# zhaoyuhsin/Edge-Guided-Near-Eye-Image-Analysis-for-Head-Mounted-Displays

Hardware: AMD Instinct MI355X
Metric: eye-frames/sec (320x240): inference edge+seg (value), +fit, exact fp32, and train fwd+bwd at 1 MI355X (higher is better)
Workload: dtype f32 tensors; inference products split into f16 hi/lo pairs (3 f16 MFMAs per product, 22-bit significand), f32 accumulate (`exact_fp32`: every product on the f32 MFMA); `train`: bf16 storage, f32 accumulate, f32 master weights (and an f32-storage leg)

## Files before the change

### edge-guided-near-eye-image-analysis-for-head-mounted-displays_amd/_lib.py

```python
import ctypes as C
import os

_HERE = os.path.dirname(os.path.abspath(__file__))
LIB_PATH = os.environ.get("EGNE_LIB") or os.path.join(_HERE, "csrc", "libegne_hip.so")

MAXSEG, MAXGROUP = 8, 3
ACT_NONE, ACT_RELU, ACT_LEAKY = 0, 1, 2

c_fp = C.c_void_p


class Seg(C.Structure):
    _fields_ = [("ptr", c_fp), ("pix_stride", C.c_int64), ("ch_off", C.c_int32), ("Cp", C.c_int32),
                ("scale", c_fp), ("shift", c_fp), ("act_in", C.c_int32), ("presplit", C.c_int32)]


class ConvDesc(C.Structure):
    _fields_ = [("B", C.c_int32), ("H", C.c_int32), ("W", C.c_int32), ("Ho", C.c_int32), ("Wo", C.c_int32),
                ("kh", C.c_int32), ("kw", C.c_int32), ("stride", C.c_int32),
                ("pad_h", C.c_int32), ("pad_w", C.c_int32), ("pad_mode", C.c_int32),
                ("ngroups", C.c_int32), ("dil", C.c_int32 * MAXGROUP),
                ("nseg", C.c_int32), ("seg", Seg * MAXSEG),
                ("Ktot", C.c_int32), ("CoutP", C.c_int32),
                ("w", c_fp), ("bias", c_fp), ("act", C.c_int32),
                ("post_scale", c_fp), ("post_shift", c_fp),
                ("residual", c_fp), ("res_pix_stride", C.c_int64), ("res_ch_off", C.c_int32),
                ("out", c_fp), ("out_pix_stride", C.c_int64), ("out_ch_off", C.c_int32),
                ("Cout_store", C.c_int32),
                ("stats_ws", c_fp), ("stats_nchunk", C.c_int32),
                ("pool_out", c_fp), ("pool_pix_stride", C.c_int64), ("pool_ch_off", C.c_int32),
                ("dyn_scale", C.c_void_p), ("absmax_out", C.c_void_p), ("dtype", C.c_int32),
                ("out_split", C.c_int32), ("out_split_scale", C.c_float), ("ovf_flag", C.c_void_p), ("f16_products", C.c_int32),
                ("mask_y", C.c_void_p), ("mask_pix_stride", C.c_int64), ("mask_ch_off", C.c_int32), ("mask_act", C.c_int32), ("mask_sums", C.c_void_p)]


class Dst(C.Structure):
    _fields_ = [("out", C.c_void_p), ("out_pix_stride", C.c_int64), ("out_ch_off", C.c_int32), ("C", C.c_int32), ("CoutP", C.c_int32),
                ("wfrag", C.c_void_p), ("residual", C.c_void_p), ("res_pix_stride", C.c_int64), ("res_ch_off", C.c_int32),
                ("mask_y", C.c_void_p), ("mask_pix_stride", C.c_int64), ("mask_ch_off", C.c_int32), ("act", C.c_int32),
                ("sums", C.c_void_p), ("res_pixels", C.c_int64)]


MAXDST = 6


class ConvQuery(C.Structure):
    _fields_ = [("dtype", C.c_int32), ("B", C.c_int32), ("H", C.c_int32), ("W", C.c_int32),
                ("kh", C.c_int32), ("kw", C.c_int32), ("stride", C.c_int32), ("pad_h", C.c_int32), ("pad_w", C.c_int32), ("pad_mode", C.c_int32),
                ("ngroups", C.c_int32), ("dil", C.c_int32 * MAXGROUP), ("nseg", C.c_int32),
                ("seg_C", C.c_int32 * MAXSEG), ("seg_Cp", C.c_int32 * MAXSEG), ("seg_ch_off", C.c_int32 * MAXSEG), ("seg_pix_stride", C.c_int64 * MAXSEG),
                ("seg_affine", C.c_int32 * MAXSEG), ("seg_planar", C.c_int32), ("seg_presplit", C.c_int32),
                ("Cout", C.c_int32), ("Cout_store", C.c_int32), ("dst_Cp", C.c_int32), ("dst_ch_off", C.c_int32), ("dst_pix_stride", C.c_int64),
                ("act", C.c_int32), ("has_post", C.c_int32), ("has_residual", C.c_int32), ("res_pix_stride", C.c_int64), ("res_ch_off", C.c_int32),
                ("split", C.c_int32), ("split1", C.c_int32), ("split_c4", C.c_int32), ("train", C.c_int32), ("dyn_scales", C.c_int32),
                ("is_dgrad", C.c_int32), ("want_stats", C.c_int32), ("want_pool", C.c_int32), ("pool_Cp", C.c_int32), ("pool_pix_stride", C.c_int64),
                ("want_scores", C.c_int32), ("up_add", C.c_int32), ("narrow_bf16_ok", C.c_int32), ("f16_products", C.c_int32), ("f16_storage", C.c_int32)]


class ConvChoice(C.Structure):
    _fields_ = [("kind", C.c_int32), ("name", C.c_char * 32), ("tail_frames", C.c_int32), ("fused_stats", C.c_int32), ("fused_pool", C.c_int32),
                ("small_ws_floats", C.c_int64)]


class BdcnTailDesc(C.Structure):
    _fields_ = [("B", C.c_int32), ("H", C.c_int32), ("W", C.c_int32),
                ("s", c_fp * 5), ("s1", c_fp * 5), ("h", C.c_int32 * 5), ("w", C.c_int32 * 5),
                ("stride", C.c_int32 * 5), ("crop", C.c_int32 * 5), ("up", c_fp * 5),
                ("fuse_w", c_fp), ("fuse_b", c_fp), ("out", c_fp * 11), ("edge_thres", C.c_int32)]


class LossDesc(C.Structure):
    _fields_ = [("B", C.c_int32), ("H", C.c_int32), ("W", C.c_int32),
                ("logits", c_fp), ("pix_stride", C.c_int64), ("ch_off", C.c_int32),
                ("target", c_fp), ("spatWts", c_fp), ("distMap", c_fp), ("cond", c_fp),
                ("pupil_center", c_fp), ("elNorm", c_fp), ("elOut", c_fp), ("alpha", C.c_float),
                ("grid_x", c_fp), ("grid_y", c_fp),
                ("partials", c_fp), ("out_terms", c_fp), ("pred_c", c_fp), ("elPred", c_fp),
                ("mask", c_fp), ("op_nchw", c_fp), ("coef", c_fp), ("dtype", C.c_int32),
                ("g_op_nchw", c_fp), ("g_pred_c", c_fp), ("g_elOut_up", c_fp)]


i32, i64, f32, vp = C.c_int32, C.c_int64, C.c_float, C.c_void_p
SIGNATURES = {
    "egne_conv2d_fwd": (i32, [C.POINTER(ConvDesc), vp]),
    "egne_pack_conv_weight": (i32, [vp, i32, i32, i32, i32, vp, i32, i32, vp, vp]),
    "egne_pack_conv_weight_frag": (i32, [vp, i32, i32, i32, i32, vp, i32, i32, vp, vp]),
    "egne_conv3x3_halo_supported": (i32, [C.POINTER(ConvDesc)]),
    "egne_conv3x3_halo_fwd": (i32, [C.POINTER(ConvDesc), vp]),
    "egne_conv3x3_smallcin_fwd": (i32, [C.POINTER(ConvDesc), vp, vp]),
    "egne_pack_conv_weight_f16x2": (i32, [vp, i32, i32, i32, i32, i32, i32, f32, vp, vp, vp]),
    "egne_conv2d_f16x3_fwd": (i32, [C.POINTER(ConvDesc), vp, vp, f32, f32, vp]),
    "egne_conv2d_f16x3_small_workspace_floats": (i64, [C.POINTER(ConvDesc)]),
    "egne_conv2d_f16x3_small_fwd": (i32, [C.POINTER(ConvDesc), vp, vp, f32, f32, vp, i64, vp]),
    "egne_pack_conv_weight_f16frag": (i32, [vp, i32, i32, i32, i32, i32, i32, f32, vp, vp, vp]),
    "egne_conv3x3_halo_f16_fwd": (i32, [C.POINTER(ConvDesc), vp, vp, f32, f32, vp]),
    "egne_conv1x1_3x3_fused_f16_fwd": (i32, [C.POINTER(ConvDesc), C.POINTER(ConvDesc), vp, vp, f32, f32, vp, vp, f32, f32, vp]),
    "egne_conv3x3c4_3x3_fused_f16_fwd": (i32, [C.POINTER(ConvDesc), C.POINTER(ConvDesc), vp, vp, f32, f32, vp, vp, f32, f32, vp]),
    "egne_msblock_dil_scores_f16_fwd": (i32, [C.POINTER(ConvDesc), vp, vp, f32, f32, vp, vp, vp, vp, i32, vp]),
    "egne_msblock_dil_f16_fwd": (i32, [C.POINTER(ConvDesc), vp, vp, f32, f32, vp]),
    "egne_conv3x3_rs_f16_fwd": (i32, [C.POINTER(ConvDesc), vp, vp, f32, f32, vp]),
    "egne_conv3x3_rw_f16_fwd": (i32, [C.POINTER(ConvDesc), vp, vp, f32, f32, vp]),
    "egne_conv1x1_pool2_f16x3_fwd": (i32, [C.POINTER(ConvDesc), vp, vp, f32, f32, vp]),
    "egne_conv1x1_f16x3_fwd": (i32, [C.POINTER(ConvDesc), vp, vp, f32, f32, vp]),
    "egne_dist_maps_workspace_bytes": (i64, [i32, i32, i32, i32]),
    "egne_dist_maps": (i32, [vp, i32, i32, i32, i32, vp, vp, vp]),
    "egne_zscore": (i32, [vp, vp, i32, i32, vp]),
    "egne_spatial_weights": (i32, [vp, i32, i32, i32, vp, vp]),
    "egne_eval_prep_workspace_bytes": (i64, [i32, i32, i32, i32, i32]),
    "egne_eval_prep": (i32, [vp, i32, i32, i32, i32, i32, i32, i32, vp, vp, vp, vp, i32, i32, vp, vp, vp, vp]),
    "egne_eval_render": (i32, [vp, i32, i32, i32, i32, i32, vp, vp, vp, i32, i32, C.c_double, i32, vp, vp, vp, vp, vp]),
    "egne_jpeg_workspace_bytes": (i64, [i32, i32, i32]),
    "egne_jpeg_encode": (i32, [vp, i32, i32, i32, vp, vp, vp, vp, i32, i32, vp, i64, vp, vp, vp, vp]),
    "egne_stamp_mask": (i32, [vp, i32, i32, i32, vp, i32, i32, i32, i32, i32, i32, i32, vp]),
    "egne_jpeg_decode_workspace_bytes": (i64, [i32, i32, i32, i32, i64, i32, i32]),
    "egne_jpeg_decode": (i32, [vp, i64, vp, i32, i32, i32, i32, i32, i32, vp, vp, vp, vp, vp, vp]),
    "egne_deepvog_loss_workspace_floats": (i64, [i32, i32, i32]),
    "egne_deepvog_loss_fwd": (i32, [vp, i64, i32, vp, vp, vp, i32, i32, i32, vp, vp, vp, vp, vp, vp]),
    "egne_deepvog_loss_bwd": (i32, [vp, i64, i32, vp, vp, vp, i32, i32, i32, vp, vp, vp, vp, i64, i32, vp]),
    "egne_affine_act": (i32, [vp, i64, i32, vp, i64, i32, i32, i64, vp, vp, i32, vp]),
    "egne_augment": (i32, [vp, vp, vp, vp, vp, vp, vp, vp, i32, i32, i32, vp]),
    "egne_augment_cv": (i32, [vp, vp, vp, vp, vp, vp, vp, vp, vp, vp, i32, i32, i32, vp]),
    "egne_loader_stage": (i32, [vp, vp, vp, i32, i32, i32, i32, i32, i32, i32, vp, vp, vp, vp, vp, vp, vp, vp, vp]),
    "egne_loader_finish": (i32, [vp, vp, vp, vp, i32, i32, vp]),
    "egne_conv3x3_smallcin_f16_fwd": (i32, [C.POINTER(ConvDesc), vp, vp, f32, f32, vp]),
    "egne_pack_conv3x3_c4_weight_f16": (i32, [vp, i32, i32, i32, f32, vp, vp, vp]),
    "egne_conv1x1_ms_f16x3_fwd": (i32, [C.POINTER(ConvDesc), vp, vp, f32, f32, vp]),
    "egne_pack_conv1x1_weight_f16x2_map": (i32, [vp, i32, i32, vp, i32, i32, f32, vp, vp, vp]),
    "egne_conv2d_f16x3_big_fwd": (i32, [C.POINTER(ConvDesc), vp, f32, f32, vp]),
    "egne_pack_conv_weight_f16img": (i32, [vp, i32, i32, i32, i32, i32, i32, f32, vp, vp]),
    "egne_conv2d_f16_big1_fwd": (i32, [C.POINTER(ConvDesc), vp, f32, f32, vp]),
    "egne_conv2d_f16_big1_supported": (i32, [C.POINTER(ConvDesc)]),
    "egne_pack_conv_weight_f16img1": (i32, [vp, i32, i32, i32, i32, i32, i32, f32, vp, vp]),
    "egne_pack_conv1x1_weight_f16": (i32, [vp, i32, i32, vp, i32, i32, f32, vp, vp, vp]),
    "egne_absmax": (i32, [vp, i64, i32, i32, i64, vp, vp]),
    "egne_absmax_f16": (i32, [vp, i64, i32, i32, i64, vp, vp]),
    "egne_norm_stats_workspace_bytes": (i64, [i32, i32, i32, i32]),
    "egne_norm_stats": (i32, [vp, i64, i32, i32, i32, i32, i32, f32, vp, vp, vp, vp, vp, vp]),
    "egne_norm_stats_finish": (i32, [vp, i32, i32, i32, i32, f32, vp, vp, vp]),
    "egne_norm_stats_finish_moments": (i32, [vp, i32, i32, i32, i32, f32, vp, vp, vp, vp, vp]),
    "egne_affine_inplace": (i32, [vp, i64, i32, i32, i64, vp, vp, vp]),
    "egne_affine": (i32, [vp, i64, i32, vp, i64, i32, i32, i64, vp, vp, vp]),
    "egne_avgpool2": (i32, [vp, i64, i32, vp, i64, i32, i32, i32, i32, i32, vp]),
    "egne_norm_act_pool2": (i32, [vp, i64, i32, vp, vp, i32, vp, i64, i32, i32, i32, i32, i32, vp]),
    "egne_maxpool2": (i32, [vp, i64, i32, vp, i64, i32, i32, i32, i32, i32, i32, i32, i32, vp]),
    "egne_maxpool2_f16": (i32, [vp, i64, i32, vp, i64, i32, i32, i32, i32, i32, i32, i32, i32, vp]),
    "egne_maxpool2_split": (i32, [vp, i64, i32, vp, i64, i32, i32, i32, i32, i32, i32, i32, i32, vp]),
    "egne_upsample2x": (i32, [vp, i64, i32, vp, i64, i32, i32, i32, i32, i32, vp]),
    "egne_upsample2x_nearest": (i32, [vp, i64, i32, vp, i64, i32, i32, i32, i32, i32, vp]),
    "egne_upsample2x_nearest_bwd": (i32, [vp, i64, i32, vp, i64, i32, i32, i32, i32, i32, vp]),
    "egne_nchw_to_nhwc": (i32, [vp, i32, i32, i32, i32, vp, i64, i32, i32, vp]),
    "egne_nhwc_to_nchw": (i32, [vp, i64, i32, i32, i32, i32, i32, vp, vp]),
    "egne_bdcn_stage_scores": (i32, [C.POINTER(vp), i32, i64, i64, vp, vp, vp, vp, vp, vp, vp, vp, vp]),
    "egne_bdcn_tail": (i32, [C.POINTER(BdcnTailDesc), vp]),
    "egne_loss_workspace_floats": (i64, [i32, i32, i32]),
    "egne_loss_fwd": (i32, [C.POINTER(LossDesc), vp]),
    "egne_selfcorr_workspace_floats": (i64, [i32, i32, i32]),
    "egne_selfcorr_fwd": (i32, [C.POINTER(LossDesc), f32, vp, vp, vp]),
    "egne_selfcorr_bwd": (i32, [C.POINTER(LossDesc), f32, vp, vp, vp, vp, vp, vp]),
    "egne_ellipse_head_act": (i32, [vp, i32, i32, vp]),
    "egne_selu_inplace": (i32, [vp, i64, vp]),
    "egne_spatial_mean": (i32, [vp, i64, i32, i32, i32, i32, vp, vp]),
    "egne_softmax3": (i32, [vp, i64, i32, vp, i64, i32, i32, i64, vp]),
    "egne_adain": (i32, [vp, i64, i32, i32, vp, vp, i64, i32, vp, i64, i32, i32, i32, f32, vp]),
    "egne_conf_loss": (i32, [vp, i32, vp, i32, i32, i32, f32, vp, vp]),
    "egne_loss_bwd": (i32, [C.POINTER(LossDesc), vp, vp, i64, i32, vp, vp]),
    "egne_act_bwd_bias_workspace_bytes": (i64, [i64, i32]),
    "egne_act_bwd_bias": (i32, [vp, i64, i32, vp, i64, i32, i32, i32, i64, vp, i32, i32, vp, vp]),
    "egne_act_bwd_bias_absmax": (i32, [vp, i64, i32, vp, i64, i32, i32, i32, i64, vp, i32, i32, vp, vp, vp]),
    "egne_act_norm_bwd": (i32, [vp, i64, i32, vp, i64, i32, i32, vp, vp, vp, i64, i32, vp, i64, i32, i32, i32, i32, i32, i32, vp, vp, vp, i32, vp, i32, vp]),
    "egne_bn_act_bwd": (i32, [vp, i64, i32, i32, vp, vp, vp, vp, i64, i32, i32, i32, i32, i32, vp, i64, i32, vp, vp, vp, vp, i32, vp, i32, vp, vp]),
    "egne_zero_many": (i32, [vp, i32, i64, vp]),
    "egne_pair_bias_bwd_workspace_bytes": (i64, [i32, i32]),
    "egne_pair_bias_bwd": (i32, [vp, i64, i32, i32, i32, i32, i32, vp, vp, i32, i32, vp, vp, vp, vp]),
    "egne_norm_bwd_workspace_bytes": (i64, [i32, i32, i32, i32]),
# ... 92 lines not shown
```

### edge-guided-near-eye-image-analysis-for-head-mounted-displays_amd/csrc/conv_f16x3.hip

```cpp
#include "common.h"
#include "kernel_util.h"
#include "split_f16.h"
#include <cstdlib>

namespace {

constexpr int KC = 32;
constexpr int LDH = 40;

__device__ __forceinline__ float act_apply(float v, int act) {
  if (act == EGNE_ACT_RELU) return fmaxf(v, 0.f);
  if (act == EGNE_ACT_LEAKY) return v > 0.f ? v : 0.01f * v;
  return v;
}

template <int WGM, int WGN, int TM, int TN, bool GROUPED, int PS = 0>
__global__ __launch_bounds__(256) void conv_f16x3_kernel(const egne_conv_desc p, const _Float16* __restrict__ whi,
                                                         const _Float16* __restrict__ wlo, float a_scale,
                                                         float out_scale, float* __restrict__ ksplit_ws) {
  egne::dyn_scales(p.dyn_scale, a_scale, out_scale);
  constexpr int BM = WGM * TM * 32, BN = WGN * TN * 32;
  constexpr int AR = BM / 32;
  constexpr int BI = (BN * 4 + 255) / 256;
  __shared__ __attribute__((aligned(16))) _Float16 lds[(2 * BM + 2 * BN) * LDH];
  _Float16* Ahi = lds;
  _Float16* Alo = Ahi + BM * LDH;
  _Float16* Bhi = Alo + BM * LDH;
  _Float16* Blo = Bhi + BN * LDH;

  const int tid = threadIdx.x, lane = tid & 63, wave = tid >> 6;
  const int li = lane & 31, lh = lane >> 5;
  const int wm = wave / WGN, wn = wave % WGN;
  const long long M = (long long)p.B * p.Ho * p.Wo;
  const long long m0 = (long long)blockIdx.x * BM;
  const int n0 = blockIdx.y * BN;
  const int T = p.kh * p.kw;
  const egne_seg sg = p.seg[0];
  const int hw = p.Ho * p.Wo;
  const int b0 = (int)(m0 / hw);
  const int frame_px = p.H * p.W;
  const long long in_left = ((long long)p.B - b0) * frame_px * sg.pix_stride * 4;
  const __amdgpu_buffer_rsrc_t rin = make_rsrc(sg.ptr + (long long)b0 * frame_px * sg.pix_stride,
                                               (unsigned)(in_left < 0x7fffffffll ? in_left : 0x7fffffffll));
  const unsigned wbytes = (unsigned)p.ngroups * T * p.CoutP * p.Ktot * 2u;
  const __amdgpu_buffer_rsrc_t rwh = make_rsrc(whi, wbytes), rwl = make_rsrc(wlo, wbytes);

  const int col4 = tid & 7, rbase = tid >> 3;
  int roff[AR], pb[AR], pyx[AR];
#pragma unroll
  for (int i = 0; i < AR; ++i) {
    const long long m = m0 + rbase + 32 * i;
    const int b = (int)(m / hw);
    const int r = (int)(m - (long long)b * hw);
    const int oy = r / p.Wo, ox = r - oy * p.Wo;
    pb[i] = m < M ? b : -1; pyx[i] = (oy << 16) | ox;
    roff[i] = ((((b - b0) * p.H + oy) * p.W + ox) * (int)sg.pix_stride + sg.ch_off) * 4 + ((PS & 2) ? (col4 >> 2) * 64 + (col4 & 3) * 16 : col4 * 16);
  }
  unsigned tapmask[AR];
  auto make_masks = [&](int g) {
    const int dil = p.dil[g];
#pragma unroll
    for (int i = 0; i < AR; ++i) {
      unsigned mk = 0;
      for (int ky = 0; ky < p.kh; ++ky)
        for (int kx = 0; kx < p.kw; ++kx) {
          const int iy = (pyx[i] >> 16) + (ky - p.pad_h) * dil, ix = (pyx[i] & 0xffff) + (kx - p.pad_w) * dil;
          if (pb[i] >= 0 && iy >= 0 && iy < p.H && ix >= 0 && ix < p.W) mk |= 1u << (ky * p.kw + kx);
        }
      tapmask[i] = mk;
    }
  };
  make_masks(0);

  int boff[BI];
#pragma unroll
  for (int j = 0; j < BI; ++j) {
    const int item = tid + 256 * j;
    const int row = item >> 2, piece = item & 3;
    boff[j] = row < BN ? ((n0 + row) * p.Ktot + piece * 8) * 2 : (int)OOB;
  }

  u32x4 ra[AR];
  u32x4 rbh[BI], rbl[BI];
  unsigned okmask = 0;
  int st_c = 0;
// ... 137 lines not shown
            const float v = acc[tm][tn][r] * out_scale + bv;
            res[tm][tn][r] += fmaxf(v, v * slope_out);
          }
          acc[tm][tn] = (f32x16)(0.f);
        }
      }
    }
    __syncthreads();
    if (more) store_step();
    __syncthreads();
    g = ng; tap = ntap; c0 = nc0;
  }

  const long long left = M - m0;
  if (!GROUPED && Z > 1) {
    float* wz = ksplit_ws + ((long long)zi * M + m0) * p.CoutP;
#pragma unroll
    for (int tn = 0; tn < TN; ++tn) {
      const int n = n0 + (wn * TN + tn) * 32 + li;
#pragma unroll
      for (int tm = 0; tm < TM; ++tm) {
        const int mrow = (wm * TM + tm) * 32 + 4 * lh;
#pragma unroll
        for (int r = 0; r < 16; ++r) {
          const int mr = mrow + (r & 3) + 8 * (r >> 2);
          if (mr < left) wz[(long long)mr * p.CoutP + n] = acc[tm][tn][r] * out_scale;
        }
      }
    }
    return;
  }
  const __amdgpu_buffer_rsrc_t rout = make_rsrc(p.out + m0 * p.out_pix_stride, (unsigned)((left < BM ? left : BM) * p.out_pix_stride * 4));
  const __amdgpu_buffer_rsrc_t rres = make_rsrc(p.residual ? p.residual + m0 * p.res_pix_stride : nullptr,
                                                p.residual ? (unsigned)((left < BM ? left : BM) * p.res_pix_stride * 4) : 0u);
  const int ostep = (int)p.out_pix_stride * 4, rstep = (int)p.res_pix_stride * 4;
  bool bad = false;
#pragma unroll
  for (int tn = 0; tn < TN; ++tn) {
    const int n = n0 + (wn * TN + tn) * 32 + li;
    const bool nok = n < p.Cout_store;
    const float bv = (!GROUPED && p.bias && nok) ? p.bias[n] : 0.f;
    float ps = 1.f, pt = 0.f;
    if (p.post_scale && nok) { ps = p.post_scale[n]; pt = p.post_shift[n]; }
#pragma unroll
    for (int tm = 0; tm < TM; ++tm) {
      const int mrow = (wm * TM + tm) * 32 + 4 * lh;
      const unsigned o0 = nok ? (unsigned)(mrow * ostep + (p.out_ch_off + n) * 4) : OOB;
      float rv[16];
#pragma unroll
      for (int r = 0; r < 16; ++r) rv[r] = 0.f;
      if (p.residual) {
        const unsigned r0 = nok ? (unsigned)(mrow * rstep + (p.res_ch_off + n) * 4) : OOB;
#pragma unroll
        for (int r = 0; r < 16; ++r)
          rv[r] = __builtin_bit_cast(float, __builtin_amdgcn_raw_buffer_load_b32(rres, (int)(r0 + ((r & 3) + 8 * (r >> 2)) * rstep), 0, 0));
      }
      if constexpr (PS & 1) {
        const unsigned s0 = nok ? (unsigned)(mrow * ostep + (p.out_ch_off + (n & ~31)) * 4 + (n & 31) * 2) : OOB;
#pragma unroll
        for (int r = 0; r < 16; r += 2) {
          float v0 = acc[tm][tn][r] * out_scale + bv, v1 = acc[tm][tn][r + 1] * out_scale + bv;
          v0 = fmaxf(v0, v0 * slope_out); v1 = fmaxf(v1, v1 * slope_out);
          h2 hh, ll;
          egne::split2(v0, v1, p.out_split_scale, hh, ll);
          if (tn == 0) bad |= egne_nonfinite(v0) || egne_nonfinite(v1) || egne_nonfinite((float)hh[0]) || egne_nonfinite((float)hh[1]);
#pragma unroll
          for (int e = 0; e < 2; ++e) {
            const int o = (int)(s0 + (((r + e) & 3) + 8 * ((r + e) >> 2)) * ostep);
            const _Float16 he = hh[e], le = ll[e];
            __builtin_amdgcn_raw_buffer_store_b16(__builtin_bit_cast(unsigned short, he), rout, o, 0, 0);
            __builtin_amdgcn_raw_buffer_store_b16(__builtin_bit_cast(unsigned short, le), rout, o + 64, 0, 0);
          }
        }
        continue;
      }
#pragma unroll
      for (int r = 0; r < 16; ++r) {
        float v;
        if (GROUPED) v = res[tm][tn][r];
        else { v = acc[tm][tn][r] * out_scale + bv; v = fmaxf(v, v * slope_out); }
        v = v * ps + pt + rv[r];
        if (tn == 0) bad |= egne_nonfinite(v);
        __builtin_amdgcn_raw_buffer_store_b32(__builtin_bit_cast(unsigned, v), rout, (int)(o0 + ((r & 3) + 8 * (r >> 2)) * ostep), 0, 0);
      }
    }
  }
  egne_ovf_commit(bad, p.ovf_flag);
}

__global__ __launch_bounds__(256) void splitk_finish_k(const egne_conv_desc p, const float* __restrict__ ws, int Z, long long M) {
  const int nq = p.CoutP / 4;
  const long long i = (long long)blockIdx.x * blockDim.x + threadIdx.x;
  if (i >= M * nq) return;
  const long long m = i / nq;
  const int n = (int)(i - m * nq) * 4;
  if (n >= p.Cout_store) return;
  f32x4 a = *(const f32x4*)(ws + m * p.CoutP + n);
  for (int z = 1; z < Z; ++z) a += *(const f32x4*)(ws + ((long long)z * M + m) * p.CoutP + n);
  const float slope = p.act == EGNE_ACT_RELU ? 0.f : (p.act == EGNE_ACT_LEAKY ? 0.01f : 1.f);
  float* o = p.out + m * p.out_pix_stride + p.out_ch_off + n;
  const float* rs = p.residual ? p.residual + m * p.res_pix_stride + p.res_ch_off + n : nullptr;
#pragma unroll
  for (int e = 0; e < 4; ++e) {
    if (n + e >= p.Cout_store) break;
    float v = a[e] + (p.bias ? p.bias[n + e] : 0.f);
    v = fmaxf(v, v * slope);
    if (p.post_scale) v = v * p.post_scale[n + e] + p.post_shift[n + e];
    if (rs) v += rs[e];
    o[e] = v;
    egne_ovf_commit(egne_nonfinite(v), p.ovf_flag);
  }
}

__global__ void pack_weight_f16x2_k(const float* __restrict__ w, int Cout, int Cin, int T, int CoutP, int Ktot,
                                    float wscale, _Float16* __restrict__ hi, _Float16* __restrict__ lo) {
  const long long total = (long long)T * CoutP * Ktot;
  for (long long i = (long long)blockIdx.x * blockDim.x + threadIdx.x; i < total; i += (long long)gridDim.x * blockDim.x) {
    const int k = (int)(i % Ktot);
    long long q = i / Ktot;
    const int n = (int)(q % CoutP);
    const int t = (int)(q / CoutP);
    float v = (n < Cout && k < Cin) ? w[((long long)n * Cin + k) * T + t] * wscale : 0.f;
    const _Float16 h = (_Float16)v;
    hi[i] = h;
    lo[i] = (_Float16)(v - (float)h);
  }
}

}

extern "C" int egne_pack_conv_weight_f16x2(const float* w_oihw, int Cout, int Cin, int kh, int kw, int CoutP, int Ktot,
                                           float wscale, void* whi, void* wlo, void* stream) {
  EGNE_REQUIRE(w_oihw && whi && wlo && Cout > 0 && Cin > 0 && CoutP >= Cout && CoutP % 32 == 0 && Ktot >= Cin && Ktot % 32 == 0,
               "pack_f16x2: bad sizes Cout %d Cin %d CoutP %d Ktot %d", Cout, Cin, CoutP, Ktot);
  long long total = (long long)kh * kw * CoutP * Ktot, g = (total + 255) / 256;
  if (g > 4096) g = 4096;
  hipLaunchKernelGGL(pack_weight_f16x2_k, dim3((unsigned)g), dim3(256), 0, (hipStream_t)stream, w_oihw, Cout, Cin, kh * kw, CoutP,
                     Ktot, wscale, (_Float16*)whi, (_Float16*)wlo);
  return egne::check_launch("egne_pack_conv_weight_f16x2");
}

namespace {

struct SmallPlan { int small, Z, wide; long long ws_floats; };

SmallPlan small_plan(const egne_conv_desc& d) {
  static const int target = [] { const char* e = getenv("EGNE_SMALL_WGS"); return e ? atoi(e) : 640; }();
  static const int wide_ok = [] { const char* e = getenv("EGNE_SMALL_WIDE"); return e ? atoi(e) : 1; }();
  static const int minsteps = [] { const char* e = getenv("EGNE_SMALL_MINSTEPS"); return e ? atoi(e) : 6; }();
  SmallPlan sp{0, 1, 0, 0};
  if (d.ngroups != 1) return sp;
  const long long M = (long long)d.B * d.Ho * d.Wo;
  const int nsteps = d.kh * d.kw * ((d.seg[0].Cp + KC - 1) / KC);
  long long tiles;
  if (d.CoutP % 128 == 0) tiles = ((M + 127) / 128) * (d.CoutP / 128);
  else if (d.CoutP % 64 == 0) tiles = ((M + 255) / 256) * (d.CoutP / 64);
  else tiles = ((M + 255) / 256) * (d.CoutP / 32);
  if (tiles >= 192) return sp;
  sp.small = 1;
  sp.wide = wide_ok && d.CoutP % 128 == 0 && nsteps >= 8 * minsteps && tiles * (nsteps / minsteps) >= target;
  const long long t2 = sp.wide ? tiles : (d.CoutP % 64 == 0 ? ((M + 63) / 64) * (d.CoutP / 64) : ((M + 127) / 128) * (d.CoutP / 32));
  int Z = (int)((target + t2 - 1) / t2);
  if (Z > nsteps / minsteps) Z = nsteps / minsteps;
  if (Z > 16) Z = 16;
  if (Z < 1) Z = 1;
  sp.Z = Z;
  sp.ws_floats = Z > 1 ? (long long)Z * M * d.CoutP : 0;
  return sp;
}

int f16x3_impl(const egne_conv_desc* dp, const void* whi, const void* wlo, float a_scale, float w_scale, float* ws, long long ws_floats,
               bool allow_small, void* stream) {
  EGNE_REQUIRE(dp && whi && wlo, "conv_f16x3: null pointer");
  const egne_conv_desc& d = *dp;
  EGNE_REQUIRE(d.nseg == 1 && d.ngroups >= 1 && d.ngroups <= EGNE_MAXGROUP && d.stride == 1 && d.pad_mode == 0 &&
               (d.seg[0].scale == nullptr) == (d.seg[0].shift == nullptr) && (d.ngroups == 1 || !d.seg[0].scale),
               "conv_f16x3: unsupported descriptor");
  EGNE_REQUIRE(d.kh >= 1 && d.kw >= 1 && d.kh * d.kw <= 32, "conv_f16x3: %d taps (%dx%d): the per-row tap mask holds 32", d.kh * d.kw, d.kh, d.kw);
  EGNE_REQUIRE(d.seg[0].Cp % 8 == 0 && (d.seg[0].Cp + 31) / 32 * 32 == d.Ktot && d.CoutP % 32 == 0,
               "conv_f16x3: Cp %d Ktot %d (must be Cp rounded up to 32) CoutP %d", d.seg[0].Cp, d.Ktot, d.CoutP);
  EGNE_REQUIRE(d.seg[0].ptr && ((uintptr_t)d.seg[0].ptr & 15) == 0 && d.seg[0].ch_off % 4 == 0 && d.seg[0].pix_stride % 4 == 0,
               "conv_f16x3: input alignment");
  EGNE_REQUIRE(((uintptr_t)whi & 15) == 0 && ((uintptr_t)wlo & 15) == 0 && d.out && d.Cout_store <= d.CoutP &&
               d.out_ch_off + d.Cout_store <= d.out_pix_stride, "conv_f16x3: weights / output");
  EGNE_REQUIRE(a_scale > 0.f && w_scale > 0.f, "conv_f16x3: scales");
  EGNE_REQUIRE((d.seg[0].presplit == 0 || d.seg[0].presplit == 3) && (d.out_split == 0 || d.out_split == 3),
               "conv_f16x3: storage (presplit %d, out_split %d): 0 or 3 (channel-order split pairs)", d.seg[0].presplit, d.out_split);
  EGNE_REQUIRE((d.out_split == 0 && d.seg[0].presplit == 0) || (!allow_small && d.ngroups == 1 && d.CoutP % 128 == 0 && d.f16_products != 1 && !d.dyn_scale && !d.seg[0].scale && !d.residual &&
                                    !d.post_scale && (d.out_split == 0 || d.out_split_scale > 0.f) && d.seg[0].Cp % 32 == 0 && d.Cout_store % 32 == 0 && d.out_ch_off % 32 == 0 &&
                                    d.out_pix_stride % 4 == 0 && (d.seg[0].presplit == 0 || d.seg[0].ch_off % 32 == 0)),
               "conv_f16x3: split-pair storage needs a plain three-product layer with CoutP %% 128 == 0 and whole 32-channel blocks");
  for (int g = 0; g < d.ngroups; ++g) {
    const int dd = d.dil[g];
    EGNE_REQUIRE(dd >= 1, "conv_f16x3: dilation");
    const int ho = d.H + 2 * d.pad_h * dd - dd * (d.kh - 1), wo = d.W + 2 * d.pad_w * dd - dd * (d.kw - 1);
    EGNE_REQUIRE(ho == d.Ho && wo == d.Wo, "conv_f16x3: output %dx%d inconsistent with geometry", d.Ho, d.Wo);
  }
  const long long M = (long long)d.B * d.Ho * d.Wo;
  const float os = 1.0f / (a_scale * w_scale);
  hipStream_t st = (hipStream_t)stream;
  const _Float16* h = (const _Float16*)whi;
  const _Float16* l = (const _Float16*)wlo;
  static const int big = [] { const char* e = getenv("EGNE_SPLIT_BIG"); return e ? atoi(e) : 0; }();
  const SmallPlan sp = allow_small ? small_plan(d) : SmallPlan{0, 1, 0, 0};
  if (sp.small) {
    EGNE_REQUIRE(sp.Z == 1 || (ws && ws_floats >= sp.ws_floats && ((uintptr_t)ws & 15) == 0), "conv_f16x3: split-K workspace too small (%lld floats, need %lld)",
                 ws_floats, sp.ws_floats);
    if (sp.wide) {
      dim3 grid((unsigned)((M + 127) / 128), (unsigned)(d.CoutP / 128), (unsigned)sp.Z);
      hipLaunchKernelGGL((conv_f16x3_kernel<2, 2, 2, 2, false>), grid, dim3(256), 0, st, d, h, l, a_scale, os, ws);
    } else if (d.CoutP % 64 == 0) {
      dim3 grid((unsigned)((M + 63) / 64), (unsigned)(d.CoutP / 64), (unsigned)sp.Z);
      hipLaunchKernelGGL((conv_f16x3_kernel<2, 2, 1, 1, false>), grid, dim3(256), 0, st, d, h, l, a_scale, os, ws);
    } else {
      dim3 grid((unsigned)((M + 127) / 128), (unsigned)(d.CoutP / 32), (unsigned)sp.Z);
      hipLaunchKernelGGL((conv_f16x3_kernel<4, 1, 1, 1, false>), grid, dim3(256), 0, st, d, h, l, a_scale, os, ws);
    }
    if (sp.Z > 1) {
      const long long items = M * (d.CoutP / 4);
      hipLaunchKernelGGL(splitk_finish_k, dim3((unsigned)((items + 255) / 256)), dim3(256), 0, st, d, ws, sp.Z, M);
    }
  } else if (d.out_split == 3 || d.seg[0].presplit == 3) {
    dim3 grid((unsigned)((M + 127) / 128), (unsigned)(d.CoutP / 128));
    if (d.seg[0].presplit == 3 && d.out_split == 3) hipLaunchKernelGGL((conv_f16x3_kernel<2, 2, 2, 2, false, 3>), grid, dim3(256), 0, st, d, h, l, a_scale, os, (float*)nullptr);
    else if (d.seg[0].presplit == 3) hipLaunchKernelGGL((conv_f16x3_kernel<2, 2, 2, 2, false, 2>), grid, dim3(256), 0, st, d, h, l, a_scale, os, (float*)nullptr);
    else hipLaunchKernelGGL((conv_f16x3_kernel<2, 2, 2, 2, false, 1>), grid, dim3(256), 0, st, d, h, l, a_scale, os, (float*)nullptr);
  } else if (d.CoutP % 128 == 0 && d.ngroups == 1 && big && M >= 256 * 512) {
    dim3 grid((unsigned)((M + 255) / 256), (unsigned)(d.CoutP / 128));
    hipLaunchKernelGGL((conv_f16x3_kernel<2, 2, 4, 2, false>), grid, dim3(256), 0, st, d, h, l, a_scale, os, (float*)nullptr);
  } else if (d.CoutP % 128 == 0 && d.ngroups == 1) {
    dim3 grid((unsigned)((M + 127) / 128), (unsigned)(d.CoutP / 128));
    hipLaunchKernelGGL((conv_f16x3_kernel<2, 2, 2, 2, false>), grid, dim3(256), 0, st, d, h, l, a_scale, os, (float*)nullptr);
  } else if (d.CoutP % 64 == 0 && d.ngroups == 1) {
    dim3 grid((unsigned)((M + 255) / 256), (unsigned)(d.CoutP / 64));
    hipLaunchKernelGGL((conv_f16x3_kernel<4, 1, 2, 2, false>), grid, dim3(256), 0, st, d, h, l, a_scale, os, (float*)nullptr);
  } else {
    dim3 grid((unsigned)((M + 255) / 256), (unsigned)(d.CoutP / 32));
    if (d.ngroups > 1) hipLaunchKernelGGL((conv_f16x3_kernel<4, 1, 2, 1, true>), grid, dim3(256), 0, st, d, h, l, a_scale, os, (float*)nullptr);
    else hipLaunchKernelGGL((conv_f16x3_kernel<4, 1, 2, 1, false>), grid, dim3(256), 0, st, d, h, l, a_scale, os, (float*)nullptr);
  }
  return egne::check_launch("egne_conv2d_f16x3_fwd");
}

}

extern "C" int egne_conv2d_f16x3_fwd(const egne_conv_desc* dp, const void* whi, const void* wlo, float a_scale,
                                     float w_scale, void* stream) {
  return f16x3_impl(dp, whi, wlo, a_scale, w_scale, nullptr, 0, false, stream);
}

extern "C" int64_t egne_conv2d_f16x3_small_workspace_floats(const egne_conv_desc* dp) {
  if (!dp) return -1;
  const SmallPlan sp = small_plan(*dp);
  return sp.small ? sp.ws_floats : -1;
}

extern "C" int egne_conv2d_f16x3_small_fwd(const egne_conv_desc* dp, const void* whi, const void* wlo, float a_scale, float w_scale,
                                           float* ws, int64_t ws_floats, void* stream) {
  return f16x3_impl(dp, whi, wlo, a_scale, w_scale, ws, ws_floats, true, stream);
}
```

### include/egne_hip.h

```cpp
#ifndef EGNE_HIP_H
#define EGNE_HIP_H

#include <stdint.h>

#ifdef __cplusplus
extern "C" {
#endif

#define EGNE_MAXSEG 8
#define EGNE_MAXGROUP 3

typedef enum {
  EGNE_OK = 0,
  EGNE_ERR_ARG = -1,
  EGNE_ERR_LAUNCH = -2,
  EGNE_ERR_NODEVICE = -3
} egne_status;

typedef enum { EGNE_ACT_NONE = 0, EGNE_ACT_RELU = 1, EGNE_ACT_LEAKY = 2 } egne_act;

typedef struct {
  const float* ptr;
  int64_t pix_stride;
  int32_t ch_off;
  int32_t Cp;
  const float* scale;
  const float* shift;
  int32_t act_in;
  int32_t presplit;
} egne_seg;

typedef struct {
  int32_t B, H, W;
  int32_t Ho, Wo;
  int32_t kh, kw, stride;
  int32_t pad_h, pad_w;
  int32_t pad_mode;
  int32_t ngroups;
  int32_t dil[EGNE_MAXGROUP];
  int32_t nseg;
  egne_seg seg[EGNE_MAXSEG];
  int32_t Ktot;
  int32_t CoutP;
  const float* w;
  const float* bias;
  int32_t act;
  const float* post_scale;
  const float* post_shift;
  const float* residual;
  int64_t res_pix_stride;
  int32_t res_ch_off;
  float* out;
  int64_t out_pix_stride;
  int32_t out_ch_off;
  int32_t Cout_store;
  double* stats_ws;
  int32_t stats_nchunk;
  float* pool_out;
  int64_t pool_pix_stride;
  int32_t pool_ch_off;
  const uint32_t* dyn_scale;
  uint32_t* absmax_out;
  int32_t dtype;
  int32_t out_split;
  float out_split_scale;
  uint32_t* ovf_flag;
  int32_t f16_products;
  const void* mask_y; int64_t mask_pix_stride; int32_t mask_ch_off; int32_t mask_act;
  float* mask_sums;
} egne_conv_desc;

int egne_conv2d_fwd(const egne_conv_desc* d, void* stream);
int egne_conv3x3_bf16_sum_rows(void);

int egne_conv3x3_halo_supported(const egne_conv_desc* d);
int egne_conv3x3_halo_fwd(const egne_conv_desc* d, void* stream);
int egne_pack_conv_weight_frag(const float* w_oihw, int Cout, int Cin, int kh, int kw,
                               const int32_t* kinv, int CoutP, int Ktot, float* w_packed, void* stream);

int egne_pack_conv_weight_f16x2(const float* w_oihw, int Cout, int Cin, int kh, int kw, int CoutP, int Ktot,
                                float wscale, void* whi, void* wlo, void* stream);
int egne_conv2d_f16x3_fwd(const egne_conv_desc* d, const void* whi, const void* wlo, float a_scale,
                          float w_scale, void* stream);
int64_t egne_conv2d_f16x3_small_workspace_floats(const egne_conv_desc* d);
int egne_conv2d_f16x3_small_fwd(const egne_conv_desc* d, const void* whi, const void* wlo, float a_scale, float w_scale,
                                float* ws, int64_t ws_floats, void* stream);

int egne_pack_conv_weight_f16img(const float* w_oihw, int Cout, int Cin, int kh, int kw, int BN, int Ktot, float wscale,
                                 void* wimg, void* stream);
int egne_conv2d_f16x3_big_fwd(const egne_conv_desc* d, const void* wimg, float a_scale, float w_scale, void* stream);
int egne_pack_conv_weight_f16img1(const float* w_oihw, int Cout, int Cin, int kh, int kw, int BN, int Ktot, float wscale,
                                  void* wimg, void* stream);
int egne_conv2d_f16_big1_supported(const egne_conv_desc* d);
int egne_conv2d_f16_big1_fwd(const egne_conv_desc* d, const void* wimg, float a_scale, float w_scale, void* stream);

int egne_pack_conv_weight_f16frag(const float* w_oihw, int Cout, int Cin, int kh, int kw, int CoutP, int Ktot,
                                  float wscale, void* fhi, void* flo, void* stream);
int egne_conv3x3_halo_f16_fwd(const egne_conv_desc* d, const void* fhi, const void* flo, float a_scale,
                              float w_scale, void* stream);

int egne_msblock_dil_f16_fwd(const egne_conv_desc* d, const void* fhi, const void* flo, float a_scale, float w_scale,
                             void* stream);
int egne_msblock_dil_scores_f16_fwd(const egne_conv_desc* d, const void* fhi, const void* flo, float a_scale, float w_scale,
                                    const float* score_w, const float* score_c, float* s0, float* s1, int accumulate,
                                    void* stream);

int egne_conv1x1_pool2_f16x3_fwd(const egne_conv_desc* d, const void* fhi, const void* flo, float a_scale, float w_scale,
                                 void* stream);

int egne_conv3x3_rs_f16_fwd(const egne_conv_desc* d, const void* fhi, const void* flo, float a_scale, float w_scale,
                            void* stream);

int egne_conv3x3_rw_f16_fwd(const egne_conv_desc* d, const void* fhi, const void* flo, float a_scale, float w_scale,
                            void* stream);

int egne_pack_conv1x1_weight_f16(const float* w_oihw, int Cout, int Cin, const int32_t* kmap, int G, int CoutP,
                                 float wscale, void* fhi, void* flo, void* stream);
int egne_conv1x1_f16x3_fwd(const egne_conv_desc* d, const void* fhi, const void* flo, float a_scale,
                           float w_scale, void* stream);

int egne_conv1x1_3x3_fused_f16_fwd(const egne_conv_desc* d1, const egne_conv_desc* d2, const void* w1hi, const void* w1lo,
                                   float a1, float w1_scale, const void* f2hi, const void* f2lo, float a2, float w2_scale,
                                   void* stream);

int egne_conv3x3c4_3x3_fused_f16_fwd(const egne_conv_desc* d1, const egne_conv_desc* d2, const void* c4hi, const void* c4lo,
                                     float a1, float w1_scale, const void* f2hi, const void* f2lo, float a2, float w2_scale,
                                     void* stream);

int egne_pack_conv1x1_weight_f16x2_map(const float* w_oihw, int Cout, int Cin, const int32_t* kmap, int CoutP, int Ktot,
                                       float wscale, void* whi, void* wlo, void* stream);
int egne_conv1x1_ms_f16x3_fwd(const egne_conv_desc* d, const void* whi, const void* wlo, float a_scale,
                              float w_scale, void* stream);

int egne_conv3x3_smallcin_fwd(const egne_conv_desc* d, const float* w40, void* stream);

int egne_pack_conv3x3_c4_weight_f16(const float* w_oihw, int Cout, int Cin, int CoutP, float wscale, void* fhi, void* flo,
                                    void* stream);
int egne_conv3x3_smallcin_f16_fwd(const egne_conv_desc* d, const void* fhi, const void* flo, float a_scale,
                                  float w_scale, void* stream);

int egne_pack_conv_weight(const float* w_oihw, int Cout, int Cin, int kh, int kw,
                          const int32_t* kinv, int CoutP, int Ktot, float* w_packed, void* stream);

int egne_absmax(const float* x, int64_t pix_stride, int ch_off, int Cp, int64_t npix, void* out_bits, void* stream);
int egne_absmax_f16(const void* x, int64_t pix_stride, int ch_off, int Cp, int64_t npix, void* out_bits, void* stream);

int64_t egne_norm_stats_workspace_bytes(int B, int HW, int Cp, int per_sample);
int egne_norm_stats(const float* x, int64_t pix_stride, int ch_off, int Cp, int B, int HW,
                    int per_sample, float eps, float* scale, float* shift,
                    float* mean_out, float* var_out, void* ws, void* stream);

int egne_norm_stats_finish(const void* ws, int Cp, int B, int nchunk, int HW, float eps, float* scale, float* shift,
                           void* stream);
int egne_norm_stats_finish_moments(const void* ws, int Cp, int B, int nchunk, int HW, float eps, float* scale, float* shift,
                                   float* mean_out, float* var_out, void* stream);

int egne_affine_inplace(float* x, int64_t pix_stride, int ch_off, int Cp, int64_t npix,
                        const float* scale, const float* shift, void* stream);

int egne_affine(const float* x, int64_t xs, int xo, float* y, int64_t ys, int yo, int Cp, int64_t npix,
                const float* scale, const float* shift, void* stream);

int egne_avgpool2(const float* x, int64_t xs, int xo, float* y, int64_t ys, int yo,
                  int B, int H, int W, int Cp, void* stream);

int egne_norm_act_pool2(const float* x, int64_t xs, int xo, const float* scale, const float* shift, int act,
// ... 382 lines not shown
```

Before: 2174.

## Add direct-to-LDS DMA pipelined kernel for presplit 3x3 f16x3 tail convs

Adds a specialised 3x3 conv kernel for presplit-input, split-output f16x3 convolutions. It loads activation and weight tiles straight into LDS with buffer/global load-to-LDS instructions, using an XOR-swizzled layout and a 2- or 3-stage ring. Padding is handled through precomputed per-row tap masks. The aim is to cut register-staged loads and overlap memory traffic with MFMA work, choosing the deeper ring when the grid fits on the CUs. This costs more dynamic LDS per block, which can lower occupancy, and adds a second code path to keep correct.

```diff
diff --git a/edge-guided-near-eye-image-analysis-for-head-mounted-displays_amd/_lib.py b/edge-guided-near-eye-image-analysis-for-head-mounted-displays_amd/_lib.py
--- a/edge-guided-near-eye-image-analysis-for-head-mounted-displays_amd/_lib.py
+++ b/edge-guided-near-eye-image-analysis-for-head-mounted-displays_amd/_lib.py
@@ -90,6 +90,7 @@
     "egne_conv3x3_smallcin_fwd": (i32, [C.POINTER(ConvDesc), vp, vp]),
     "egne_pack_conv_weight_f16x2": (i32, [vp, i32, i32, i32, i32, i32, i32, f32, vp, vp, vp]),
     "egne_conv2d_f16x3_fwd": (i32, [C.POINTER(ConvDesc), vp, vp, f32, f32, vp]),
+    "egne_conv2d_f16x3_tail_dma": (i32, [C.POINTER(ConvDesc)]),
     "egne_conv2d_f16x3_small_workspace_floats": (i64, [C.POINTER(ConvDesc)]),
     "egne_conv2d_f16x3_small_fwd": (i32, [C.POINTER(ConvDesc), vp, vp, f32, f32, vp, i64, vp]),
     "egne_pack_conv_weight_f16frag": (i32, [vp, i32, i32, i32, i32, i32, i32, f32, vp, vp, vp]),
diff --git a/edge-guided-near-eye-image-analysis-for-head-mounted-displays_amd/csrc/conv_f16x3.hip b/edge-guided-near-eye-image-analysis-for-head-mounted-displays_amd/csrc/conv_f16x3.hip
--- a/edge-guided-near-eye-image-analysis-for-head-mounted-displays_amd/csrc/conv_f16x3.hip
+++ b/edge-guided-near-eye-image-analysis-for-head-mounted-displays_amd/csrc/conv_f16x3.hip
@@ -1,6 +1,7 @@
 #include "common.h"
 #include "kernel_util.h"
 #include "split_f16.h"
+#include "tail_dma_map.h"
 #include <cstdlib>
 
 namespace {
@@ -304,6 +305,148 @@
         v = v * ps + pt + rv[r];
         if (tn == 0) bad |= egne_nonfinite(v);
         __builtin_amdgcn_raw_buffer_store_b32(__builtin_bit_cast(unsigned, v), rout, (int)(o0 + ((r & 3) + 8 * (r >> 2)) * ostep), 0, 0);
+      }
+    }
+  }
+  egne_ovf_commit(bad, p.ovf_flag);
+}
+
+template <int NST>
+__global__ __launch_bounds__(256) void conv_f16x3_tail_dma_kernel(const egne_conv_desc p, const _Float16* __restrict__ whi,
+                                                                  const _Float16* __restrict__ wlo, float out_scale) {
+  namespace tdm = egne_tdm;
+  static_assert(NST == 2 || NST == 3, "ring depth");
+  constexpr int BM = tdm::ROWS, BN = tdm::ROWS, NP = tdm::PIECES;
+  extern __shared__ __attribute__((aligned(1024))) char tdm_lds[];
+  const int tid = threadIdx.x, lane = tid & 63;
+  const int wave = __builtin_amdgcn_readfirstlane(tid >> 6);
+  const int li = lane & 31, lh = lane >> 5;
+  const int wm = wave >> 1, wn = wave & 1;
+  const long long M = (long long)p.B * p.Ho * p.Wo;
+  const long long m0 = (long long)blockIdx.x * BM;
+  const int n0 = blockIdx.y * BN;
+  const int T = p.kh * p.kw;
+  const egne_seg sg = p.seg[0];
+  const int hw = p.Ho * p.Wo, frame_px = p.H * p.W;
+  const int b0 = (int)(m0 / hw);
+  const long long in_left = ((long long)p.B - b0) * frame_px * sg.pix_stride * 4;
+  const __amdgpu_buffer_rsrc_t rin = make_rsrc(sg.ptr + (long long)b0 * frame_px * sg.pix_stride,
+                                               (unsigned)(in_left < 0x7fffffffll ? in_left : 0x7fffffffll));
+  const int dil = p.dil[0];
+
+  int roff[NP];
+  unsigned tapmask[NP];
+  const char* wsrc[NP];
+#pragma unroll
+  for (int i = 0; i < NP; ++i) {
+    const int row = tdm::piece_row(wave, i, lane), c = tdm::piece_chunk(wave, i, lane);
+    const long long m = m0 + row;
+    const int b = (int)(m / hw);
+    const int r = (int)(m - (long long)b * hw);
+    const int oy = r / p.Wo, ox = r - oy * p.Wo;
+    roff[i] = ((((b - b0) * p.H + oy) * p.W + ox) * (int)sg.pix_stride + sg.ch_off) * 4 + tdm::a_src_byte(c);
+    unsigned mk = 0;
+    for (int ky = 0; ky < p.kh; ++ky)
+      for (int kx = 0; kx < p.kw; ++kx) {
+        const int iy = oy + (ky - p.pad_h) * dil, ix = ox + (kx - p.pad_w) * dil;
+        if (m < M && iy >= 0 && iy < p.H && ix >= 0 && ix < p.W) mk |= 1u << (ky * p.kw + kx);
+      }
+    tapmask[i] = mk;
+    wsrc[i] = (const char*)(tdm::chunk_plane(c) ? wlo : whi) + ((long long)(n0 + row) * p.Ktot + tdm::b_src_half(c)) * 2;
+  }
+
+  int tap_n = 0, ky_n = 0, kx_n = 0, c0_n = 0;
+  auto load_step = [&](int stage) {
+    const int tapoff = (((ky_n - p.pad_h) * p.W + (kx_n - p.pad_w)) * dil * (int)sg.pix_stride + c0_n) * 4;
+    const long long wstep = ((long long)tap_n * p.CoutP * p.Ktot + c0_n) * 2;
+    char* sa = tdm_lds + tdm::stage_byte(stage, 0);
+    char* sb = tdm_lds + tdm::stage_byte(stage, 1);
+#pragma unroll
+    for (int i = 0; i < NP; ++i) {
+      const bool ok = (tapmask[i] >> tap_n) & 1u;
+      __builtin_amdgcn_raw_ptr_buffer_load_lds(rin, (lds_ptr)(sa + tdm::piece_lds_base(wave, i)), 16, ok ? roff[i] + tapoff : (int)OOB, 0, 0, 0);
+    }
+#pragma unroll
+    for (int i = 0; i < NP; ++i)
+      __builtin_amdgcn_global_load_lds((const __attribute__((address_space(1))) void*)(wsrc[i] + wstep), (lds_ptr)(sb + tdm::piece_lds_base(wave, i)), 16, 0, 0);
+    if (++kx_n == p.kw) { kx_n = 0; ++ky_n; }
+    if (++tap_n == T) { tap_n = 0; ky_n = 0; c0_n += 32; }
+  };
+
+  f32x16 acc[2][2];
+#pragma unroll
+  for (int a = 0; a < 2; ++a)
+#pragma unroll
+    for (int b = 0; b < 2; ++b) acc[a][b] = (f32x16)(0.f);
+
+  int fo[2][2];
+#pragma unroll
+  for (int ks = 0; ks < 2; ++ks)
+#pragma unroll
+    for (int pl = 0; pl < 2; ++pl) fo[ks][pl] = tdm::frag_lane_byte(li, ks, lh, pl);
+
+  const int nsteps = T * (sg.Cp >> 5);
+  for (int s = 0; s < NST - 1 && s < nsteps; ++s) load_step(s);
+  int st = 0, st_ld = NST - 1;
+  for (int step = 0; step < nsteps; ++step) {
+    if (NST == 3 && step + 1 < nsteps) asm volatile("s_waitcnt vmcnt(8) lgkmcnt(0)" ::: "memory");
+    else asm volatile("s_waitcnt vmcnt(0) lgkmcnt(0)" ::: "memory");
+    __builtin_amdgcn_s_barrier();
+    asm volatile("" ::: "memory");
+    if (step + NST - 1 < nsteps) load_step(st_ld);
+    const char* sa = tdm_lds + tdm::stage_byte(st, 0) + tdm::frag_block_byte(2 * wm);
+    const char* sb = tdm_lds + tdm::stage_byte(st, 1) + tdm::frag_block_byte(2 * wn);
+#pragma unroll
+    for (int ks = 0; ks < 2; ++ks) {
+      h8 ah[2], al[2], bh[2], bl[2];
+#pragma unroll
+      for (int t = 0; t < 2; ++t) {
+        ah[t] = *(const h8*)(sa + tdm::frag_block_byte(t) + fo[ks][0]);
+        al[t] = *(const h8*)(sa + tdm::frag_block_byte(t) + fo[ks][1]);
+        bh[t] = *(const h8*)(sb + tdm::frag_block_byte(t) + fo[ks][0]);
+        bl[t] = *(const h8*)(sb + tdm::frag_block_byte(t) + fo[ks][1]);
+      }
+#pragma unroll
+      for (int tm = 0; tm < 2; ++tm)
+#pragma unroll
+        for (int tn = 0; tn < 2; ++tn) {
+          acc[tm][tn] = __builtin_amdgcn_mfma_f32_32x32x16_f16(al[tm], bh[tn], acc[tm][tn], 0, 0, 0);
+          acc[tm][tn] = __builtin_amdgcn_mfma_f32_32x32x16_f16(ah[tm], bl[tn], acc[tm][tn], 0, 0, 0);
+          acc[tm][tn] = __builtin_amdgcn_mfma_f32_32x32x16_f16(ah[tm], bh[tn], acc[tm][tn], 0, 0, 0);
+        }
+    }
+    st = st + 1 == NST ? 0 : st + 1;
+    st_ld = st_ld + 1 == NST ? 0 : st_ld + 1;
+  }
+
+  const float slope_out = p.act == EGNE_ACT_RELU ? 0.f : (p.act == EGNE_ACT_LEAKY ? 0.01f : 1.f);
+  const long long left = M - m0;
+  const __amdgpu_buffer_rsrc_t rout = make_rsrc(p.out + m0 * p.out_pix_stride, (unsigned)((left < BM ? left : BM) * p.out_pix_stride * 4));
+  const int ostep = (int)p.out_pix_stride * 4;
+  bool bad = false;
+#pragma unroll
+  for (int tn = 0; tn < 2; ++tn) {
+    const int n = n0 + (wn * 2 + tn) * 32 + li;
+    const bool nok = n < p.Cout_store;
+    const float bv = (p.bias && nok) ? p.bias[n] : 0.f;
+#pragma unroll
+    for (int tm = 0; tm < 2; ++tm) {
+      const int mrow = (wm * 2 + tm) * 32 + 4 * lh;
+      const unsigned s0 = nok ? (unsigned)(mrow * ostep + (p.out_ch_off + (n & ~31)) * 4 + (n & 31) * 2) : OOB;
+#pragma unroll
+      for (int r = 0; r < 16; r += 2) {
+        float v0 = acc[tm][tn][r] * out_scale + bv, v1 = acc[tm][tn][r + 1] * out_scale + bv;
+        v0 = fmaxf(v0, v0 * slope_out); v1 = fmaxf(v1, v1 * slope_out);
+        h2 hh, ll;
+        egne::split2(v0, v1, p.out_split_scale, hh, ll);
+        if (tn == 0) bad |= egne_nonfinite(v0) || egne_nonfinite(v1) || egne_nonfinite((float)hh[0]) || egne_nonfinite((float)hh[1]);
+#pragma unroll
+        for (int e = 0; e < 2; ++e) {
+          const int o = (int)(s0 + (((r + e) & 3) + 8 * ((r + e) >> 2)) * ostep);
+          const _Float16 he = hh[e], le = ll[e];
+          __builtin_amdgcn_raw_buffer_store_b16(__builtin_bit_cast(unsigned short, he), rout, o, 0, 0);
+          __builtin_amdgcn_raw_buffer_store_b16(__builtin_bit_cast(unsigned short, le), rout, o + 64, 0, 0);
+        }
       }
     }
   }
@@ -389,6 +532,12 @@
   sp.Z = Z;
   sp.ws_floats = Z > 1 ? (long long)Z * M * d.CoutP : 0;
   return sp;
+}
+
+constexpr int TAIL_DMA_CUS = 256;
+
+bool tail_dma_takes(const egne_conv_desc& d) {
+  return d.nseg == 1 && d.ngroups == 1 && d.seg[0].presplit == 3 && d.out_split == 3 && d.kh == 3 && d.kw == 3 && (d.dil[0] == 1 || d.dil[0] == 2);
 }
 
 int f16x3_impl(const egne_conv_desc* dp, const void* whi, const void* wlo, float a_scale, float w_scale, float* ws, long long ws_floats,
@@ -444,7 +593,16 @@
     }
   } else if (d.out_split == 3 || d.seg[0].presplit == 3) {
     dim3 grid((unsigned)((M + 127) / 128), (unsigned)(d.CoutP / 128));
-    if (d.seg[0].presplit == 3 && d.out_split == 3) hipLaunchKernelGGL((conv_f16x3_kernel<2, 2, 2, 2, false, 3>), grid, dim3(256), 0, st, d, h, l, a_scale, os, (float*)nullptr);
+    if (tail_dma_takes(d)) {
+      static_assert(egne_tdm::MAX_STAGES == 3, "ring depth");
+      const bool deep = (long long)grid.x * grid.y <= TAIL_DMA_CUS;
+      const int lds_bytes = (deep ? 3 : 2) * egne_tdm::STAGE_BYTES;
+      if (!egne::raise_lds((const void*)conv_f16x3_tail_dma_kernel<2>, 2 * egne_tdm::STAGE_BYTES) ||
+          !egne::raise_lds((const void*)conv_f16x3_tail_dma_kernel<3>, 3 * egne_tdm::STAGE_BYTES))
+        return egne::fail(EGNE_ERR_LAUNCH, "conv_f16x3: cannot raise the dynamic LDS limit");
+      if (deep) hipLaunchKernelGGL((conv_f16x3_tail_dma_kernel<3>), grid, dim3(256), lds_bytes, st, d, h, l, os);
+      else hipLaunchKernelGGL((conv_f16x3_tail_dma_kernel<2>), grid, dim3(256), lds_bytes, st, d, h, l, os);
+    } else if (d.seg[0].presplit == 3 && d.out_split == 3) hipLaunchKernelGGL((conv_f16x3_kernel<2, 2, 2, 2, false, 3>), grid, dim3(256), 0, st, d, h, l, a_scale, os, (float*)nullptr);
     else if (d.seg[0].presplit == 3) hipLaunchKernelGGL((conv_f16x3_kernel<2, 2, 2, 2, false, 2>), grid, dim3(256), 0, st, d, h, l, a_scale, os, (float*)nullptr);
     else hipLaunchKernelGGL((conv_f16x3_kernel<2, 2, 2, 2, false, 1>), grid, dim3(256), 0, st, d, h, l, a_scale, os, (float*)nullptr);
   } else if (d.CoutP % 128 == 0 && d.ngroups == 1 && big && M >= 256 * 512) {
@@ -471,6 +629,8 @@
   return f16x3_impl(dp, whi, wlo, a_scale, w_scale, nullptr, 0, false, stream);
 }
 
+extern "C" int egne_conv2d_f16x3_tail_dma(const egne_conv_desc* dp) { return dp && tail_dma_takes(*dp) ? 1 : 0; }
+
 extern "C" int64_t egne_conv2d_f16x3_small_workspace_floats(const egne_conv_desc* dp) {
   if (!dp) return -1;
   const SmallPlan sp = small_plan(*dp);
diff --git a/edge-guided-near-eye-image-analysis-for-head-mounted-displays_amd/csrc/tail_dma_map.h b/edge-guided-near-eye-image-analysis-for-head-mounted-displays_amd/csrc/tail_dma_map.h
--- /dev/null
+++ b/edge-guided-near-eye-image-analysis-for-head-mounted-displays_amd/csrc/tail_dma_map.h
@@ -0,0 +1,35 @@
+#pragma once
+
+#if defined(__HIPCC__) || defined(__CUDACC__)
+#define EGNE_TDM_HD __host__ __device__ inline
+#else
+#define EGNE_TDM_HD inline
+#endif
+
+namespace egne_tdm {
+
+constexpr int ROWS = 128;
+constexpr int ROWB = 128;
+constexpr int WAVES = 4, LANES = 64;
+constexpr int PIECES = ROWS * ROWB / 16 / (WAVES * LANES);
+constexpr int OPERAND_BYTES = ROWS * ROWB;
+constexpr int STAGE_BYTES = 2 * OPERAND_BYTES;
+constexpr int MAX_STAGES = 3;
+
+EGNE_TDM_HD int key(int row) { return ((row >> 1) + 6) & 7; }
+
+EGNE_TDM_HD int piece_row(int wave, int i, int lane) { return 32 * wave + 8 * i + (lane >> 3); }
+EGNE_TDM_HD int piece_lds_base(int wave, int i) { return wave * 4096 + i * 1024; }
+EGNE_TDM_HD int piece_lds_byte(int wave, int i, int lane) { return piece_lds_base(wave, i) + lane * 16; }
+EGNE_TDM_HD int piece_chunk(int wave, int i, int lane) { return (lane & 7) ^ key(piece_row(wave, i, lane)); }
+EGNE_TDM_HD int chunk_plane(int c) { return c & 1; }
+EGNE_TDM_HD int chunk_k(int c) { return (c >> 1) * 8; }
+EGNE_TDM_HD int a_src_byte(int c) { return chunk_plane(c) * 64 + chunk_k(c) * 2; }
+EGNE_TDM_HD int b_src_half(int c) { return chunk_k(c); }
+
+EGNE_TDM_HD int stage_byte(int stage, int operand) { return stage * STAGE_BYTES + operand * OPERAND_BYTES; }
+
+EGNE_TDM_HD int frag_lane_byte(int li, int ks, int lh, int plane) { return li * ROWB + (((2 * (2 * ks + lh) + plane) ^ key(li)) << 4); }
+EGNE_TDM_HD int frag_block_byte(int blk) { return blk * 32 * ROWB; }
+
+}
diff --git a/include/egne_hip.h b/include/egne_hip.h
--- a/include/egne_hip.h
+++ b/include/egne_hip.h
@@ -82,6 +82,7 @@
                                 float wscale, void* whi, void* wlo, void* stream);
 int egne_conv2d_f16x3_fwd(const egne_conv_desc* d, const void* whi, const void* wlo, float a_scale,
                           float w_scale, void* stream);
+int egne_conv2d_f16x3_tail_dma(const egne_conv_desc* d);
 int64_t egne_conv2d_f16x3_small_workspace_floats(const egne_conv_desc* d);
 int egne_conv2d_f16x3_small_fwd(const egne_conv_desc* d, const void* whi, const void* wlo, float a_scale, float w_scale,
                                 float* ws, int64_t ws_floats, void* stream);
```

Result: no change. 2179 (median of 6 runs) (+0.2%).
